# DmSM-1/C-OFDM

Hardware: AMD Instinct MI355X
Metric: IQ-samples/sec (tx IFFT+CP and rx FFT+equalise), 2048-subcarrier frames, 1/2/4/8 GPU (higher is better)
Workload: dtype f64

## Files before the change

c-ofdm_amd/csrc/ofdm_capi.cpp:

```cpp
#include <dlfcn.h>
#include <hip/hip_runtime.h>

#include <algorithm>
#include <climits>
#include <cctype>
#include <cmath>
#include <complex>
#include <cstdarg>
#include <cstdio>
#include <cstdlib>
#include <chrono>
#include <mutex>
#include <cstring>
#include <fstream>
#include <iterator>
#include <random>
#include <stdexcept>
#include <string>
#include <unordered_map>
#include <vector>

#include "../../include/ofdm_mi355x.h"

#if __has_include(<rccl/rccl.h>)
// ... 78 lines not shown
}

}

struct ofdm_ctx {
    ofdm_params p{};
    int device = 0;
    int logn = 0;
    int N = 0, D = 0, P = 0, cp = 0, S = 0, k = 0, L = 0, seg = 0, npr = 0, t2 = 0;
    ofdm_geometry geo{};
    std::vector<cd> t2_symbol, ofdm_preamble, mod_preamble, templ;
    std::vector<uint8_t> preamble_bytes;
    std::vector<double> t2_mask;
    double2* d_tw = nullptr;
    int* d_data_bin = nullptr;
    int* d_data_slot = nullptr;
    int* d_pilot_bin = nullptr;
    int* d_bin_map = nullptr;
    int* d_rx_pack = nullptr;
    int* d_pilot_swz = nullptr;
    int* d_tx_code = nullptr;
    double2* d_const = nullptr;
    double2* d_const_bpsk = nullptr;
    double2* d_header = nullptr;
    double2* d_preamble = nullptr;
    double2* d_templ = nullptr;
    double2* d_tspec = nullptr;
    float2* d_tspec32 = nullptr;
    double2* d_twm = nullptr;
    double tspec_max = 0.0;
    double2* d_modpre = nullptr;
    double* d_t2mask = nullptr;
    double2* d_t2tw = nullptr;
    int* d_first = nullptr;
    int t2_logn = -1;
    struct CfoPlan {
        int nsym = 0, logm = -1, g = 0;
        double2* tw_sub = nullptr;
        double2* tw_full = nullptr;
        int* borders = nullptr;
    };
    std::vector<CfoPlan> cfo_plans;
    double* d_cfo_scratch = nullptr;
    size_t cfo_scratch_n = 0;
    double2* d_scratch = nullptr;
    size_t scratch_bytes = 0;
// ... 278 lines not shown
                data_slot[d] = jj;
                bin_map[segst[jj] + t] = d;
            }
        }
    }
    std::vector<int> rx_pack(std::max(c->D, ofdm::RX_DPT * (c->N / 8)), 0),
        pilot_swz(std::max(c->P, c->N / 8), 0);
    for (int d = 0; d < c->D; ++d) rx_pack[d] = ofdm::lds_swz_host(data_bin[d]) | (data_slot[d] << 16);
    for (int j = 0; j < c->P; ++j) pilot_swz[j] = ofdm::lds_swz_host(pilot[j]);
    std::vector<int> tx_code(c->N);
    for (int b = 0; b < c->N; ++b)
        tx_code[b] = bin_map[b] >= 0 ? ofdm::tx_code_data(bin_map[b])
                                     : ofdm::tx_code_fixed(bin_map[b] == -2 ? ofdm::TX_LDS_PILOT : ofdm::TX_LDS_ZERO);
    if ((rc = upload(&c->d_rx_pack, rx_pack)) || (rc = upload(&c->d_pilot_swz, pilot_swz)) ||
        (rc = upload(&c->d_tx_code, tx_code)) ||
        (rc = upload(&c->d_tw, twiddles(c->N))) || (rc = upload(&c->d_data_bin, data_bin)) ||
        (rc = upload(&c->d_data_slot, data_slot)) || (rc = upload(&c->d_pilot_bin, pilot)) ||
        (rc = upload(&c->d_bin_map, bin_map)) || (rc = upload(&c->d_const, constellation(c->k))) ||
        (rc = upload(&c->d_const_bpsk, constellation(1)))) {
        ofdm_destroy(c);
        return rc;
    }

    c->t2_symbol.assign(c->t2, cd(0, 0));
    if (c->t2) {
        std::vector<cd> spec(c->t2, cd(0, 0));
        spec[params->t2_sin_f1] = cd(0.5, 0);
        spec[params->t2_sin_f2] = cd(0.5, 0);
        for (int n = 0; n < c->t2; ++n) {
            cd acc(0, 0);
            for (int kk = 0; kk < c->t2; ++kk) {
                if (spec[kk] == cd(0, 0)) continue;
                const double a = 2.0 * M_PI * (double)(((long)kk * n) % c->t2) / (double)c->t2;
                acc += spec[kk] * cd(std::cos(a), std::sin(a));
            }
            c->t2_symbol[n] = acc;
        }
    }
    c->t2_mask.assign(std::max(1, c->t2), 0.0);
    if (c->t2) {
        const int sm = (int)params->smooth, f1 = (int)params->t2_sin_f1, f2 = (int)params->t2_sin_f2;
        for (int i = std::max(0, f1 - sm); i <= std::min(c->t2 - 1, f1 + sm); ++i) c->t2_mask[i] += 1.0;
        for (int i = std::max(0, f2 - sm); i <= std::min(c->t2 - 1, f2 + sm); ++i) c->t2_mask[i] += 1.0;
    }

    {
// ... 193 lines not shown
    const int pilot_w = int(S * rel_pilot_w);
    std::vector<int> borders(P + 2);
    for (int i = 0, j = int((1.0 - rel_bw - rel_pilot_w) / 2.0 * S); i < P + 2; i++) {
        borders[i] = j;
        j += pilot_w;
    }
    borders[0] = std::max(0, borders[0]);
    for (int b : borders)
        if (b < 0 || b > S) return fail(OFDM_ERR_UNSUPPORTED, "pilot_freq_sinh windows leave the spectrum");
    int rc;
    if ((rc = upload(&pl.tw_sub, twiddles(1 << pl.logm))) || (rc = upload(&pl.borders, borders))) return rc;
    if (pl.g == 5 && (rc = upload(&pl.tw_full, twiddles((int)S)))) return rc;
    c->cfo_plans.push_back(pl);
    *out = &c->cfo_plans.back();
    return OFDM_OK;
}

int ofdm_get_geometry(const ofdm_ctx* c, ofdm_geometry* o)
{
    if (!c || !o) return fail(OFDM_ERR_INVALID, "null argument");
    *o = c->geo;
    return OFDM_OK;
}

int ofdm_get_t2_symbol(const ofdm_ctx* c, double* o)
{
    if (!c || !o) return fail(OFDM_ERR_INVALID, "null argument");
    std::memcpy(o, c->t2_symbol.data(), c->t2_symbol.size() * sizeof(cd));
    return OFDM_OK;
}

int ofdm_get_preamble(const ofdm_ctx* c, uint8_t* bytes, double* pre, double* modp, double* templ)
{
    if (!c) return fail(OFDM_ERR_INVALID, "null ctx");
    if (bytes) std::memcpy(bytes, c->preamble_bytes.data(), c->preamble_bytes.size());
    if (pre) std::memcpy(pre, c->ofdm_preamble.data(), c->ofdm_preamble.size() * sizeof(cd));
    if (modp) std::memcpy(modp, c->mod_preamble.data(), c->mod_preamble.size() * sizeof(cd));
    if (templ) std::memcpy(templ, c->templ.data(), c->templ.size() * sizeof(cd));
    return OFDM_OK;
}

int ofdm_device_alloc(ofdm_ctx* c, size_t bytes, void** d)
{
    if (!c || !d) return fail(OFDM_ERR_INVALID, "null argument");
    HIP_TRY(hipSetDevice(c->device));
    HIP_TRY(hipMalloc(d, std::max<size_t>(bytes, 1)));
// ... 205 lines not shown
    if (nframes > 0x7fffffffu) return fail(OFDM_ERR_INVALID, "too many frames in one call");
    ofdm::RxArgs a{};
    a.tab = c->tables(false);
    a.iq = iq16 ? nullptr : reinterpret_cast<const double2*>(iq);
    a.iq16 = reinterpret_cast<const short2*>(iq16);
    a.nframes = (long)nframes;
    a.frame_stride = (long)frame_stride;
    a.chan = reinterpret_cast<const double2*>(chan);
    a.chan_stride = (long)chan_stride;
    a.constell = reinterpret_cast<double2*>(constell_out);
    a.read_out = reinterpret_cast<double2*>(read_out);
    a.bytes = bytes_out;
    a.ref = ref_bytes;
    a.bit_errors = bit_errors;
    a.S = c->S;
    a.D = c->D;
    a.P = c->P;
    a.seg = c->seg;
    a.cp = c->cp;
    a.k = c->k;
    a.bytes_per_frame = c->geo.bytes_per_frame;
    a.pilot_ampl = (double)c->p.pilot_ampl / 1000;
    a.queue = rx_queue(c, (hipStream_t)stream);
    const bool fits = c->S <= ofdm::RX_SMAX && c->D <= ofdm::RX_DPT * (c->N / 8);
    if (!fits) {
        if (c->D > ofdm::RX_DPT * (c->N / 8))
            return fail(OFDM_ERR_UNSUPPORTED, "num_data_subc > fft_size/2 is not covered by the rx kernel");
        if (constell_out) {
            a.ystage = a.constell;
        } else {
            const size_t need = nframes * (size_t)c->S * c->D * sizeof(double2);
            if (need > c->scratch_bytes) {
                if (capturing((hipStream_t)stream)) return capture_refused("growing the staged rx scratch");
                HIP_TRY(hipSetDevice(c->device));
                if (c->d_scratch) HIP_TRY(hipFree(c->d_scratch));
                c->d_scratch = nullptr;
                c->scratch_bytes = 0;
                HIP_TRY(hipMalloc((void**)&c->d_scratch, need));
                c->scratch_bytes = need;
            }
            a.ystage = c->d_scratch;
        }
    }
    hipError_t e = soft ? ofdm::launch_rx_soft(c->logn, a, *soft, (hipStream_t)stream)
                        : ofdm::launch_rx(c->logn, a, (hipStream_t)stream, nullptr);
    if (e != hipSuccess) {
// ... 1429 lines not shown
```

c-ofdm_amd/csrc/ofdm_dev.hpp:

```cpp
#pragma once
#include <hip/hip_runtime.h>
#include <cstdint>
#include <mutex>
#include <set>
#include <utility>

#include "ofdm_fft.hpp"

namespace ofdm {

inline void lds_opt_in(const void* fn, int bytes)
{
    static std::mutex mu;
    static std::set<std::pair<const void*, int>> done;
    int dev = 0;
    if (hipGetDevice(&dev) != hipSuccess) dev = 0;
    std::lock_guard<std::mutex> g(mu);
    if (done.insert({fn, dev}).second)
        (void)hipFuncSetAttribute(fn, hipFuncAttributeMaxDynamicSharedMemorySize, bytes);
}

__device__ __forceinline__ int decide_select(double2 z, int k, double s1, int m)
{
    const double re = __builtin_fmin(__builtin_fmax(z.x, -1.0), 1.0);
    const double im = __builtin_fmin(__builtin_fmax(z.y, -1.0), 1.0);
    const int ire = (uint8_t)(int)add_rn(mul_rn(add_rn(re, 1.0), s1), 0.5);
    const int iim = (uint8_t)(int)add_rn(mul_rn(add_rn(im, 1.0), s1), 0.5);
    const int qam = (ire | (iim * m)) & 0xff;
    const int bpsk = (z.x + z.y) > 0.0;
    return k == 1 ? bpsk : qam;
}

enum { LLR_F32 = 0, LLR_I8 = 1 };

struct SoftScale {
    double c, h1;
    int h;
};

__device__ __forceinline__ SoftScale soft_scale(int k, double s)
{
    SoftScale q;
    q.h = k >> 1;
    q.h1 = (double)((1 << q.h) - 1) * 0.5;
    q.c = k == 1 ? -2.8284271247461903 * s : s / (q.h1 * q.h1);
    return q;
}

template <int H>
__device__ __forceinline__ void soft_axis(double x, double s1, const SoftScale& q, double (&L)[4])
{
#pragma unroll
    for (int b = 0; b < 4; ++b) L[b] = 0.0;
// ... 162 lines not shown
```

c-ofdm_amd/csrc/ofdm_internal.hpp:

```cpp
#pragma once
#include <hip/hip_runtime.h>
#include <cstdint>

namespace ofdm {

struct DevTables {
    const double2* tw;
    const int* data_bin;
    const int* data_slot;
    const int* pilot_bin;
    const int* bin_map;
    const int* rx_pack;
    const int* pilot_swz;
    const int* tx_code;
    const double2* constell;
};

struct TxArgs {
    DevTables tab;
    const uint8_t* bytes;
    const double2* points;
    double2* iq;
    int16_t* iq16;
    const double2* header;
// ... 17 lines not shown
struct RxArgs {
    DevTables tab;
    const double2* iq;
    const short2* iq16;
    long nframes;
    long frame_stride;
    const double2* chan;
    long chan_stride;
    bool chan_recip;
    double2* constell;
    double2* read_out;
    uint8_t* bytes;
    const uint8_t* ref;
    unsigned long long* bit_errors;
    double2* ystage;
    const long* starts;
    long start_off;
    const long* count;
    int* queue;
    const double2* corr;
    int S, D, P, seg, cp, k;
    long bytes_per_frame;
    double pilot_ampl;
};

struct SoftArgs {
    void* llr;
    const double* frame_scale;
    double scale;
    int fmt;
};

hipError_t launch_rx_soft(int logn, const RxArgs& a, const SoftArgs& sa, hipStream_t stream);
hipError_t launch_soft_demap(const double2* pts, long n, int k, double scale, int fmt, void* out, hipStream_t stream);
hipError_t launch_tx(int logn, const TxArgs& a, hipStream_t stream);
hipError_t launch_rx(int logn, const RxArgs& a, hipStream_t stream, bool* staged_needed);
hipError_t launch_copy(void* dst, const void* src, size_t n, hipStream_t stream);
hipError_t launch_demap(double2* pts, long n, int k, uint8_t* bytes, hipStream_t stream);
hipError_t launch_map(const uint8_t* bytes, long nbytes, int k, const double2* table, double2* out,
                      hipStream_t stream);
hipError_t launch_bit_convert(const uint8_t* in, long len, int in_bits, int out_bits, uint8_t* out, long out_len,
                              hipStream_t stream);
hipError_t launch_i16_to_f64(const int16_t* in, long n, double* out, hipStream_t stream);
hipError_t launch_f64_to_i16(const double* in, long n, double mult, int16_t* out, hipStream_t stream);

constexpr int RX_SMAX = 8;
inline int lds_swz_host(int e) { return e ^ ((e >> 3) & 7); }
constexpr int RX_DPT = 4;
constexpr int RX_WAVES_PER_CU = 8;
constexpr int TX_LDS_PILOT = 256, TX_LDS_ZERO = 257;
inline int tx_code_data(int d) { return d | (0xff << 13); }
inline int tx_code_fixed(int entry) { return entry << 21; }
constexpr long TX_MAX_GRID = 4096;


struct FecRate { int period, kept; unsigned mask; };
__host__ __device__ inline FecRate fec_rate(int rate)
{
    return rate == 0 ? FecRate{1, 1, 0x1u} : rate == 1 ? FecRate{4, 3, 0x7u} : FecRate{6, 4, 0x27u};
// ... 58 lines not shown
```

c-ofdm_amd/csrc/ofdm_kernels.hip:

```cpp
#include <hip/hip_runtime.h>
#include <algorithm>
#include <cstdint>
#include <cstdlib>

#include "ofdm_dev.hpp"
#include "ofdm_fft.hpp"
#include "ofdm_internal.hpp"
#include "ofdm_rx2.hpp"

#include <type_traits>

namespace ofdm {


__device__ __forceinline__ int symbol_bits(const uint8_t* __restrict__ b, long nbytes, long g, int k)
{
    const long bit = g * k;
    const long byte = bit >> 3;
    const int off = (int)(bit & 7);
    const int mask = (1 << k) - 1;
    if (off + k <= 8) return (b[byte] >> (8 - off - k)) & mask;
    const int w = ((int)b[byte] << 8) | (byte + 1 < nbytes ? (int)b[byte + 1] : 0);
    return (w >> (16 - off - k)) & mask;
}
// ... 798 lines not shown
            lds_opt_in((const void*)rx_wide_kernel<LOGN>, 160 * 1024);
            hipLaunchKernelGGL(rx_wide_kernel<LOGN>, dim3((unsigned)a.nframes), dim3(a.S * FS::T),
                               rx_wide_shm<LOGN>(a), st, a);
            return hipGetLastError();
        }
    }
    return fits ? rx_launch_n<LOGN, false, false, false>(a, st) : rx_launch_n<LOGN, true, false, false>(a, st);
}

hipError_t launch_rx(int logn, const RxArgs& a, hipStream_t st, bool* staged)
{
    switch (logn) {
        case 6: return rx_dispatch<6>(a, st, staged);
        case 7: return rx_dispatch<7>(a, st, staged);
        case 8: return rx_dispatch<8>(a, st, staged);
        case 9: return rx_dispatch<9>(a, st, staged);
        case 10: return rx_dispatch<10>(a, st, staged);
        case 11: return rx_dispatch<11>(a, st, staged);
        case 12: return rx_dispatch<12>(a, st, staged);
        default: return hipErrorInvalidValue;
    }
}

hipError_t launch_demap(double2* pts, long n, int k, uint8_t* bytes, hipStream_t st)
{
    const long nbytes = (n * k + 7) / 8;
    if (nbytes <= 0) return hipSuccess;
    const int bs = 256;
    hipLaunchKernelGGL(demap_kernel, dim3((unsigned)((nbytes + bs - 1) / bs)), dim3(bs), 0, st, pts, n, k, bytes,
                       nbytes);
    return hipGetLastError();
}

hipError_t launch_soft_demap(const double2* pts, long n, int k, double scale, int fmt, void* out, hipStream_t st)
{
    if (n <= 0) return hipSuccess;
    const long ntiles = (n + 1023) / 1024;
    const long cap = 8L * num_cus();
    const unsigned grid = (unsigned)(ntiles < cap ? ntiles : cap);
    if (fmt == LLR_F32)
        hipLaunchKernelGGL(soft_demap_kernel<LLR_F32>, dim3(grid), dim3(256), 0, st, pts, n, k, scale, out);
    else
        hipLaunchKernelGGL(soft_demap_kernel<LLR_I8>, dim3(grid), dim3(256), 0, st, pts, n, k, scale, out);
    return hipGetLastError();
}

// ... 113 lines not shown
```

c-ofdm_amd/csrc/ofdm_rx_body.inc:

```
    using FS = FftShape<LOGN>;
    constexpr int N = FS::N, T = FS::T;
    constexpr int SW = STAGED ? 1 : RX_SMAX;
    extern __shared__ double2 smem[];
    const int S0 = a.S, P0 = a.P;
    double2* bufA = smem;
    double2* bufB = bufA + N;
    double2* lds_tw = bufB + FS::PADN;
    double2* pil = lds_tw + TwLds<LOGN>::SIZE;
    double2* gain = pil + S0 * P0;
    double* red = reinterpret_cast<double*>(gain + S0 * P0);
    uint8_t* dec = reinterpret_cast<uint8_t*>(bufA);

    const int t0 = threadIdx.x;
    const int L = N + a.cp;
    const long fstep = gridDim.x;
    const long fbase = (SYNC && a.nframes > 0 && (!a.count || *a.count > 0) && a.starts[0] < 0) ? 1 : 0;
    const long nfr = (a.count ? min(*a.count, a.nframes) : a.nframes) - fbase;
    auto leave = [&]() {
        if (a.queue && threadIdx.x == 0) {
            __threadfence();
            if (atomicAdd(a.queue + 1, 1) == (int)gridDim.x - 1) {
                a.queue[0] = 0;
                a.queue[1] = 0;
            }
// ... 8 lines not shown
    constexpr bool kTwSplit = T >= TwLds<LOGN>::SIZE;
    TwPiece<LOGN> twp{};
    if constexpr (kTwSplit)
        twp = tw_fetch<LOGN>(a.tab.tw, t0);
    else
        load_twiddles<LOGN>(a.tab.tw, lds_tw, t0, T);
    int pk[RX_DPT];
#pragma unroll
    for (int i = 0; i < RX_DPT; ++i) pk[i] = a.tab.rx_pack[t0 + T * i];
    const int pbin = a.tab.pilot_swz[t0];
    long fl = blockIdx.x;
    auto frame_of = [&](long l) { return l + fbase; };
    SymbolRegs<LOGN, I16> pf;
    auto body0 = [&](long g) { return SYNC ? a.starts[g] + a.start_off : g * a.frame_stride + a.cp; };
    dma_symbol<LOGN, I16>(a, body0(frame_of(fl)), bufB, t0);
    if constexpr (kTwSplit) tw_store<LOGN>(twp, lds_tw);
    lds_barrier();

    unsigned long long errs = 0;

#pragma unroll 1
    for (long fnext; fl < nfr; fl = fnext) {
        const long f = frame_of(fl);
        int t;
        asm volatile("v_mov_b32 %0, %1" : "=v"(t) : "v"(t0));
#pragma unroll
        for (int i = 0; i < RX_DPT; ++i) asm volatile("" : "+v"(pk[i]));
        int S = a.S, D = a.D, P = a.P;
        asm volatile("" : "+s"(S), "+s"(D), "+s"(P));
        const long x0 = body0(f);
        const int m = 1 << (a.k / 2);
        const double s1 = a.k == 1 ? 0.0 : 1.0 / (2.0 / (m - 1));
        const bool whole_frame_dec = (long)S * D <= (long)FS::PADN * 16;
        const long bpf = a.bytes_per_frame;
        const bool by_word = (a.k == 1 || a.k == 2 || a.k == 4 || a.k == 8) && (bpf & 3) == 0 &&
                             ((uintptr_t)a.bytes & 3) == 0 && ((uintptr_t)a.ref & 3) == 0;
        SoftScale sq{};
        char* llr_f = nullptr;
        int llr_esz = 0;
        bool llr_vec = false;
        if constexpr (SOFT) {
            sq = soft_scale(a.k, sa.frame_scale ? sa.scale * sa.frame_scale[f] : sa.scale);
            llr_esz = sa.fmt == LLR_F32 ? 4 : 1;
            llr_f = static_cast<char*>(sa.llr) + f * S * D * a.k * llr_esz;
            llr_vec = ((uintptr_t)sa.llr & 15) == 0;
        }
// ... 36 lines not shown
            if (t < P) pil[s * P + t] = res[pbin];
            if constexpr (STAGED) {
#pragma unroll
                for (int i = 0; i < RX_DPT; ++i) {
                    const int d = t + T * i;
                    if (d < D) a.ystage[(f * S + s) * D + d] = res[pk[i] & 0xffff];
                }
            } else {
                switch (s) {
#define OFDM_RX_PUT(W)                                                                    \
    case W:                                                                               \
        if constexpr (W < SW) {                                                           \
            _Pragma("unroll") for (int i = 0; i < RX_DPT; ++i) y[W][i] = res[pk[i] & 0xffff]; \
        }                                                                                 \
        break;
                    OFDM_RX_PUT(0) OFDM_RX_PUT(1) OFDM_RX_PUT(2) OFDM_RX_PUT(3)
                    OFDM_RX_PUT(4) OFDM_RX_PUT(5) OFDM_RX_PUT(6) OFDM_RX_PUT(7)
#undef OFDM_RX_PUT
                    default: break;
                }
            }
        }
        lds_barrier();
        const double2* chan = a.chan ? a.chan + f * a.chan_stride : nullptr;
        const int dec_b = (S * D + 15) & ~15;
        double2* chl = reinterpret_cast<double2*>(reinterpret_cast<char*>(bufA) + dec_b);
        const bool chan_lds = chan && dec_b + D * 16 <= N * 16;
        if (chan_lds) dma_chan<LOGN>(chan, D, chl, t);
        const bool early = !a.queue;
        if (early) {
            fnext = fl + fstep;
            if (fnext < nfr) dma_symbol<LOGN, I16>(a, body0(frame_of(fnext)), bufB, t);
        }
        int qv = 0;
        if (a.queue && t == 0) qv = atomicAdd(a.queue, 1);

        double acc = 0.0;
        for (int i = t; i < S * P; i += T) acc += hypot(pil[i].x, pil[i].y);
        acc = block_sum_lds<T>(acc, red);
        const double phys = acc / ((double)(P * S) * a.pilot_ampl);

        for (int i = t; i < S * P; i += T) {
            const int j = i % P;
            const double2 c0 = make_double2(pil[j].x / phys, pil[j].y / phys);
            const double2 cs = make_double2(pil[i].x / phys, pil[i].y / phys);
            const double2 coef = cdiv_exact(cs, c0);
            const double2 g = cdiv_exact(make_double2(1.0, 0.0), coef);
            gain[i] = make_double2(g.x / phys, g.y / phys);
        }
        if (chan_lds) {
            if (early && fnext < nfr)
                asm volatile("s_waitcnt vmcnt(8)" ::: "memory");
            else
                asm volatile("s_waitcnt vmcnt(0)" ::: "memory");
        }
        if (a.queue && t == 0) *qslot = qv;
        lds_barrier();
        if (!early) {
            fnext = fstep + __builtin_amdgcn_readfirstlane(*qslot);
            if (fnext < nfr) dma_symbol<LOGN, I16>(a, body0(frame_of(fnext)), bufB, t);
        }

        auto emit_point = [&](int s, int i, double2 yv) {
            int d = t + T * i, gi = s * P + (pk[i] >> 16);
            asm volatile("" : "+v"(d), "+v"(gi));
            double2 o = cmul_exact(yv, gain[gi]);
            if (a.read_out) store_nt(a.read_out + (f * S + s) * D + d, o);
            const double2 cv = chan_lds ? chl[d] : load_untracked(chan + d);
            o = a.chan_recip ? cmul_exact(o, cv) : cdiv_exact(o, cv);
            if (a.constell) store_nt(a.constell + (f * S + s) * D + d, o);
            if constexpr (SOFT)
                soft_emit(o, a.k, s1, sq, sa.fmt, llr_f + (long)(s * D + d) * (a.k * llr_esz), llr_vec);
            dec[whole_frame_dec ? s * D + d : d] = (uint8_t)decide(o, a.k, s1, m);
// ... 2 lines not shown
            double2* cbase = a.constell + (f * S + s) * D;
#pragma unroll
            for (int i = 0; i < RX_DPT; ++i) {
                int d = t + T * i, gi = s * P + (pk[i] >> 16);
                asm volatile("" : "+v"(d), "+v"(gi));
                if (d < D) {
                    const double2 o = cmul_exact(yw[i], gain[gi]);
                    if constexpr (decltype(with_store)::value) store_nt(cbase + d, o);
                    if constexpr (SOFT)
                        soft_emit(o, a.k, s1, sq, sa.fmt, llr_f + (long)(s * D + d) * (a.k * llr_esz), llr_vec);
                    dec[whole_frame_dec ? s * D + d : d] = (uint8_t)decide_select(o, a.k, s1, m);
                }
            }
        };
        auto emit_group = [&](int s, const double2 (&yw)[RX_DPT]) {
            if (SYNC || chan) {
#pragma unroll
                for (int i = 0; i < RX_DPT; ++i)
                    if (t + T * i < D) emit_point(s, i, yw[i]);
            } else if (a.constell) {
                emit_plain(s, yw, std::true_type{});
            } else {
                emit_plain(s, yw, std::false_type{});
            }
        };

        auto pack = [&](long jb0, long jb1, long dbase) {
            for (long jb = jb0 + t; jb < jb1; jb += T) {
                int byte = 0;
                if (a.k == 1 || a.k == 2 || a.k == 4 || a.k == 8) {
                    const int per = 8 / a.k;
                    const long p0 = (jb - jb0) * per + dbase;
                    for (int r = 0; r < per; ++r) byte = (byte << a.k) | dec[p0 + r];
                } else {
                    for (int b = 0; b < 8; ++b) {
                        const long bit = (jb - jb0) * 8 + b;
                        const long g = bit / a.k + dbase;
                        const int within = (int)(bit % a.k);
                        byte = (byte << 1) | ((dec[g] >> (a.k - 1 - within)) & 1);
                    }
                }
                if (a.bytes) a.bytes[f * bpf + jb] = (uint8_t)byte;
                if (a.ref) errs += __popc((unsigned)(byte ^ a.ref[f * bpf + jb]));
            }
        };

        auto pack_words = [&]() {
            const int per_word = 32 / a.k;
            for (long w = t; w < bpf / 4; w += T) {
                const uint8_t* dw = dec + w * per_word;
                uint32_t word;
                switch (a.k) {
                    case 1: word = pack_word<1>(dw); break;
                    case 2: word = pack_word<2>(dw); break;
                    case 4: word = pack_word<4>(dw); break;
                    default: word = pack_word<8>(dw); break;
                }
                if (a.bytes) reinterpret_cast<uint32_t*>(a.bytes + f * bpf)[w] = word;
                if (a.ref) errs += __popc(word ^ reinterpret_cast<const uint32_t*>(a.ref + f * bpf)[w]);
            }
        };

        if constexpr (!STAGED) {
#pragma unroll 1
            for (int w = 0; w < S; ++w) {
                if constexpr (SOFT) {
                    double2 yw[RX_DPT] = {};
                    switch (w) {
#define OFDM_RX_TAKE(W)                                                        \
    case W:                                                                    \
        if constexpr (W < SW) {                                                \
            _Pragma("unroll") for (int i = 0; i < RX_DPT; ++i) yw[i] = y[W][i]; \
        }                                                                      \
        break;
                        OFDM_RX_TAKE(0) OFDM_RX_TAKE(1) OFDM_RX_TAKE(2) OFDM_RX_TAKE(3)
                        OFDM_RX_TAKE(4) OFDM_RX_TAKE(5) OFDM_RX_TAKE(6) OFDM_RX_TAKE(7)
#undef OFDM_RX_TAKE
                        default: break;
                    }
                    emit_group(w, yw);
                    continue;
                }
                switch (w) {
#define OFDM_RX_EMIT(W)                 \
    case W:                             \
        if constexpr (W < SW) {         \
            emit_group(w, y[W]);        \
        }                               \
        break;
                    OFDM_RX_EMIT(0) OFDM_RX_EMIT(1) OFDM_RX_EMIT(2) OFDM_RX_EMIT(3)
                    OFDM_RX_EMIT(4) OFDM_RX_EMIT(5) OFDM_RX_EMIT(6) OFDM_RX_EMIT(7)
#undef OFDM_RX_EMIT
                    default: break;
                }
            }
            lds_barrier();
            if (by_word)
                pack_words();
            else
                pack(0, bpf, 0);
        } else {
            const long bps = (long)D * a.k / 8;
            for (int s = 0; s < S; ++s) {
                double2 yst[RX_DPT];
#pragma unroll
                for (int i = 0; i < RX_DPT; ++i)
                    yst[i] = t + T * i < D ? a.ystage[(f * S + s) * D + t + T * i] : make_double2(0.0, 0.0);
                emit_group(s, yst);
                lds_barrier();
                if (!whole_frame_dec) {
                    pack(s * bps, (s + 1) * bps, 0);
                    lds_barrier();
                }
            }
            if (whole_frame_dec) pack(0, bpf, 0);
        }
        lds_barrier();
    }
    if (a.bit_errors) {
        errs = block_sum_u64<T>(errs, red);
        if (t0 == 0 && errs) atomicAdd(a.bit_errors, errs);
    }
    leave();
```

c-ofdm_amd/devtest/ofdm_devtest.hip:

```cpp
#include <hip/hip_runtime.h>

#include "../csrc/ofdm_syncdev.hpp"

namespace {

__global__ void atan2_kernel(const double* __restrict__ y, const double* __restrict__ x, double* __restrict__ out,
                             long n)
{
    const long i = (long)blockIdx.x * blockDim.x + threadIdx.x;
    if (i < n) out[i] = ofdm::atan2_fast(y[i], x[i]);
}

__global__ void cp_phase_kernel(const double2* __restrict__ acc, const double2* __restrict__ rot,
                                double* __restrict__ out, long n)
{
    const long i = (long)blockIdx.x * blockDim.x + threadIdx.x;
    if (i < n) out[i] = ofdm::cp_phase(acc[i], rot[i]);
}

template <int NT, bool WAVE>
__global__ void __launch_bounds__(WAVE ? 2 * NT : NT)
unwrap_kernel(double* __restrict__ ph, const int* __restrict__ len, long stride)
{
    __shared__ double lds[4 * NT + 1];
    __shared__ unsigned scr[(NT + 63) / 64];
    double* row = ph + (long)blockIdx.x * stride;
    const int n = min(len[blockIdx.x], 4 * NT + 1);
    for (int i = threadIdx.x; i < n; i += blockDim.x) lds[i] = row[i];
    __syncthreads();
    if (!WAVE || threadIdx.x < NT) ofdm::unwrap_scan<NT, WAVE>(lds, n, scr);
    __syncthreads();
    for (int i = threadIdx.x; i < n; i += blockDim.x) row[i] = lds[i];
}

template <int NT, bool WAVE>
int launch_unwrap(double* ph, const int* len, int nseq, long stride, hipStream_t s)
{
    hipLaunchKernelGGL((unwrap_kernel<NT, WAVE>), dim3(nseq), dim3(WAVE ? 2 * NT : NT), 0, s, ph, len, stride);
    return (int)hipGetLastError();
}

}

extern "C" {

int ofdm_devtest_atan2(const double* y, const double* x, double* out, long n, hipStream_t s)
{
    if (n <= 0) return 0;
    hipLaunchKernelGGL(atan2_kernel, dim3((unsigned)((n + 255) / 256)), dim3(256), 0, s, y, x, out, n);
    return (int)hipGetLastError();
}

int ofdm_devtest_cp_phase(const double* acc, const double* rot, double* out, long n, hipStream_t s)
{
    if (n <= 0) return 0;
    hipLaunchKernelGGL(cp_phase_kernel, dim3((unsigned)((n + 255) / 256)), dim3(256), 0, s,
                       reinterpret_cast<const double2*>(acc), reinterpret_cast<const double2*>(rot), out, n);
    return (int)hipGetLastError();
}

int ofdm_devtest_unwrap(int nt, int wave, double* ph, const int* len, int nseq, long stride, hipStream_t s)
{
    if (nseq <= 0) return 0;
    if (stride < 4L * nt + 1) return -1;
    if (wave) return nt == 64 ? launch_unwrap<64, true>(ph, len, nseq, stride, s) : -1;
    switch (nt) {
    case 8: return launch_unwrap<8, false>(ph, len, nseq, stride, s);
// ... 10 lines not shown
```

c-ofdm_amd/python/ofdm_mi355x.py:

```python
from __future__ import annotations

import ctypes as C
import os
import subprocess

HERE = os.path.dirname(os.path.abspath(__file__))
PKG = os.path.dirname(HERE)
LIB_PATH = os.environ.get("OFDM_MI355X_LIB") or os.path.join(PKG, "lib", "libofdm_mi355x.so")
HEADER = os.path.join(os.path.dirname(PKG), "include", "ofdm_mi355x.h")

PARAM_FIELDS = [
    "fft_size", "num_data_subc", "num_pilot_subc", "cp_size", "num_symb", "num_pr_symb",
    "pr_sin_len", "pr_seed", "pr_level", "t2sin_size", "t2_sin_f1", "t2_sin_f2",
    "t2_sin_level", "smooth", "mod_type", "pilot_ampl", "mult", "rx_buf_size", "iterations",
]

OFDM_OK = 0
ERRORS = {-1: "INVALID", -2: "UNSUPPORTED", -3: "HIP", -4: "IO", -5: "NOMEM", -6: "PARSE"}
LLR_F32, LLR_I8 = 0, 1
FEC_R12, FEC_R23, FEC_R34 = 0, 1, 2
IL_FORWARD, IL_INVERSE = 0, 1
SYNC_CFO, SYNC_FREQ_SHIFT, SYNC_CP, SYNC_PHASE, SYNC_CHAN, SYNC_ALL = 1, 2, 4, 8, 16, 31


# ... 30 lines not shown


class WalkState(C.Structure):
    _fields_ = [("pos", C.c_long), ("ring_end", C.c_long)]


class OfdmError(RuntimeError):
    def __init__(self, code: int, msg: str):
        super().__init__(f"ofdm error {code} ({ERRORS.get(code, '?')}): {msg}")
        self.code = code


_V, _I, _L, _SZ, _D = C.c_void_p, C.c_int, C.c_long, C.c_size_t, C.c_double
_PP = C.POINTER(Params)
SIGNATURES = {
    "ofdm_last_error": (C.c_char_p, []),
    "ofdm_abi_version": (_I, []),
    "ofdm_params_default": (_I, [_PP]),
    "ofdm_params_from_config": (_I, [C.c_char_p, _PP]),
    "ofdm_config_lookup": (_I, [C.c_char_p, C.c_char_p, C.POINTER(C.c_long)]),
    "ofdm_create": (_I, [_PP, _I, C.POINTER(_V)]),
    "ofdm_destroy": (_I, [_V]),
    "ofdm_get_geometry": (_I, [_V, C.POINTER(Geometry)]),
    "ofdm_get_t2_symbol": (_I, [_V, _V]),
    "ofdm_get_preamble": (_I, [_V, _V, _V, _V, _V]),
    "ofdm_device_alloc": (_I, [_V, _SZ, C.POINTER(_V)]),
    "ofdm_device_free": (_I, [_V, _V]),
    "ofdm_memcpy_h2d": (_I, [_V, _V, _V, _SZ, _V]),
    "ofdm_memcpy_d2h": (_I, [_V, _V, _V, _SZ, _V]),
    "ofdm_copy": (_I, [_V, _V, _V, _SZ, _V]),
    "ofdm_rx_demod_read": (_I, [_V, _V, _SZ, _SZ, _V, _SZ, _V, _V, _V, _V]),
    "ofdm_memset_device": (_I, [_V, _V, _I, _SZ, _V]),
    "ofdm_stream_synchronize": (_I, [_V, _V]),
    "ofdm_tx_modulate": (_I, [_V, _V, _SZ, _V, _SZ, _V, C.POINTER(Channel), _V]),
    "ofdm_tx_frames": (_I, [_V, _V, _SZ, _V, _V, _V]),
    "ofdm_rx_demod": (_I, [_V, _V, _SZ, _SZ, _V, _SZ, _V, _V, _V, _V, _V]),
    "ofdm_rx_demod_i16": (_I, [_V, _V, _SZ, _SZ, _V, _SZ, _V, _V, _V, _V, _V]),
    "ofdm_demap": (_I, [_V, _V, _SZ, _V, _V]),
    "ofdm_soft_demap": (_I, [_V, _V, _SZ, _D, _I, _V, _V]),
    "ofdm_rx_demod_soft": (_I, [_V, _V, _V, _SZ, _SZ, _V, _SZ, _D, _V, _I, _V, _V, _V, _V, _V, _V]),
    "ofdm_chan_estimate_ls": (_I, [_V, _V, _SZ, _SZ, _I, _V, _SZ, _V, _SZ, _V]),
    "ofdm_soft_demap_csi": (_I, [_V, _V, _SZ, _V, _SZ, _D, _V, _I, _V, _V]),
    "ofdm_fec_coded_bits": (_I, [_SZ, _I, C.POINTER(_SZ)]),
    "ofdm_fec_max_info_bits": (_I, [_SZ, _I, C.POINTER(_SZ)]),
    "ofdm_fec_workspace_size": (_I, [_SZ, _SZ, C.POINTER(_SZ)]),
    "ofdm_fec_encode": (_I, [_V, _V, _SZ, _SZ, _SZ, _I, _V, _SZ, _V]),
# ... 133 lines not shown
    def __init__(self, params, device: int = 0):
        if isinstance(params, dict):
            params = Params.make(**params)
        self.params = params
        self.device = device
        h = C.c_void_p()
        check(lib().ofdm_create(C.byref(params), device, C.byref(h)))
        self.h = h
        g = Geometry()
        check(lib().ofdm_get_geometry(h, C.byref(g)))
        self.geo = g

    def close(self):
        if getattr(self, "h", None):
            lib().ofdm_destroy(self.h)
            self.h = None

    def __del__(self):
        try:
            self.close()
        except Exception:
            pass

    def t2_symbol(self):
        import numpy as np
        out = np.zeros(self.params.t2sin_size, np.complex128)
        check(lib().ofdm_get_t2_symbol(self.h, out.ctypes.data))
        return out

    def preamble(self):
        import numpy as np
        p = self.params
        b = np.zeros(p.num_data_subc * p.num_pr_symb // 8, np.uint8)
        pre = np.zeros(self.geo.preamble_len, np.complex128)
        modp = np.zeros(p.num_data_subc * p.num_pr_symb, np.complex128)
        tpl = np.zeros(p.pr_sin_len, np.complex128)
        check(lib().ofdm_get_preamble(self.h, b.ctypes.data, pre.ctypes.data, modp.ctypes.data,
                                      tpl.ctypes.data))
        return b, pre, modp, tpl

    def tx(self, data, nframes: int, iq_out, frame_stride: int | None = None, iq16_out=None,
           noise_std: float = 0.0, seed: int = 0, sample_offset: int = 0, stream=None):
        stride = self.geo.message_len if frame_stride is None else frame_stride
        ch = Channel(noise_std, seed, sample_offset) if noise_std > 0 else None
        check(lib().ofdm_tx_modulate(self.h, _ptr(data), nframes, _ptr(iq_out), stride,
                                     _ptr(iq16_out), C.byref(ch) if ch else None, _stream(stream)))
# ... 237 lines not shown
```

include/ofdm_mi355x.h:

```cpp
#ifndef OFDM_MI355X_H
#define OFDM_MI355X_H

#include <stddef.h>
#include <stdint.h>

#ifdef __cplusplus
extern "C" {
#endif

#define OFDM_MI355X_ABI_VERSION 5

enum {
    OFDM_OK = 0,
    OFDM_ERR_INVALID = -1,
    OFDM_ERR_UNSUPPORTED = -2,
    OFDM_ERR_HIP = -3,
    OFDM_ERR_IO = -4,
    OFDM_ERR_NOMEM = -5,
    OFDM_ERR_PARSE = -6
};

typedef struct ofdm_params {
    long fft_size;
    long num_data_subc;
// ... 27 lines not shown
    long segment_size;
    long pilot_bin[256];
    long segment_bin[256];
} ofdm_geometry;

typedef struct ofdm_channel {
    double noise_std;
    unsigned long long seed;
    unsigned long long sample_offset;
} ofdm_channel;

typedef struct ofdm_ctx ofdm_ctx;

const char* ofdm_last_error(void);
int ofdm_abi_version(void);

int ofdm_params_default(ofdm_params* out);
int ofdm_params_from_config(const char* path, ofdm_params* out);
int ofdm_config_lookup(const char* path, const char* key, long* value);

int ofdm_create(const ofdm_params* params, int device, ofdm_ctx** out);
int ofdm_destroy(ofdm_ctx* ctx);
int ofdm_get_geometry(const ofdm_ctx* ctx, ofdm_geometry* out);
int ofdm_get_t2_symbol(const ofdm_ctx* ctx, double* out );
int ofdm_get_preamble(const ofdm_ctx* ctx,
                      uint8_t* bytes_out ,
                      double* ofdm_preamble_out ,
                      double* mod_preamble_out ,
                      double* template_out );

int ofdm_device_alloc(ofdm_ctx* ctx, size_t bytes, void** dptr);
int ofdm_device_free(ofdm_ctx* ctx, void* dptr);
int ofdm_memcpy_h2d(ofdm_ctx* ctx, void* dst, const void* src, size_t bytes, void* stream);
int ofdm_memcpy_d2h(ofdm_ctx* ctx, void* dst, const void* src, size_t bytes, void* stream);
int ofdm_memset_device(ofdm_ctx* ctx, void* dst, int value, size_t bytes, void* stream);
int ofdm_stream_synchronize(ofdm_ctx* ctx, void* stream);
int ofdm_host_alloc(ofdm_ctx* ctx, size_t bytes, void** hptr);
int ofdm_host_free(ofdm_ctx* ctx, void* hptr);
int ofdm_stream_create(ofdm_ctx* ctx, void** stream);
int ofdm_stream_destroy(ofdm_ctx* ctx, void* stream);
int ofdm_memcpy_d2d(ofdm_ctx* ctx, void* dst, const void* src, size_t bytes, void* stream);
int ofdm_copy(ofdm_ctx* ctx, void* dst, const void* src, size_t bytes, void* stream);
int ofdm_event_create(ofdm_ctx* ctx, void** event);
int ofdm_event_record(ofdm_ctx* ctx, void* event, void* stream);
int ofdm_event_synchronize(ofdm_ctx* ctx, void* event);
int ofdm_event_destroy(ofdm_ctx* ctx, void* event);
// ... 188 lines not shown
```

Before: 142.1 billion.

## Add fast QPSK rx emit path with threshold decisions and DPP word packing

Adds a fast receive emit path for QPSK without per-frame channel input. At create time a one-off device scan finds decision thresholds that match the existing decide_select bit for bit and validates them, then enables the path. In that path hard decisions become simple compares, and bits are packed into 32-bit words with cross-lane DPP moves and written directly, replacing the LDS staging, barrier and separate pack pass. Reference bytes are DMA'd into LDS for the bit-error count. This adds complexity and leaves the path off for other modulations or when validation fails.

```diff
diff --git a/c-ofdm_amd/csrc/ofdm_capi.cpp b/c-ofdm_amd/csrc/ofdm_capi.cpp
--- a/c-ofdm_amd/csrc/ofdm_capi.cpp
+++ b/c-ofdm_amd/csrc/ofdm_capi.cpp
@@ -124,6 +124,8 @@
     int* d_tx_code = nullptr;
     double2* d_const = nullptr;
     double2* d_const_bpsk = nullptr;
+    double dec_tau[3] = {};
+    bool dec_fast = false;
     double2* d_header = nullptr;
     double2* d_preamble = nullptr;
     double2* d_templ = nullptr;
@@ -448,6 +450,21 @@
         return rc;
     }
 
+    if (c->k == 2) {
+        double* d_tau = nullptr;
+        double h_tau[4] = {};
+        hipError_t e = hipMalloc((void**)&d_tau, sizeof(h_tau));
+        if (e == hipSuccess) e = ofdm::launch_decide_tau_scan(c->k, d_tau, nullptr);
+        if (e == hipSuccess) e = hipMemcpy(h_tau, d_tau, sizeof(h_tau), hipMemcpyDeviceToHost);
+        if (d_tau) (void)hipFree(d_tau);
+        if (e != hipSuccess) {
+            ofdm_destroy(c);
+            return hip_fail(e, "decision threshold scan");
+        }
+        for (int j = 0; j < 3; ++j) c->dec_tau[j] = h_tau[j];
+        c->dec_fast = h_tau[3] == 1.0;
+    }
+
     c->t2_symbol.assign(c->t2, cd(0, 0));
     if (c->t2) {
         std::vector<cd> spec(c->t2, cd(0, 0));
@@ -687,6 +704,8 @@
     *o = c->geo;
     return OFDM_OK;
 }
+
+int ofdm_rx_emit_fast(const ofdm_ctx* c) { return c ? (c->dec_fast ? 1 : 0) : -1; }
 
 int ofdm_get_t2_symbol(const ofdm_ctx* c, double* o)
 {
@@ -938,6 +957,8 @@
     a.bytes_per_frame = c->geo.bytes_per_frame;
     a.pilot_ampl = (double)c->p.pilot_ampl / 1000;
     a.queue = rx_queue(c, (hipStream_t)stream);
+    for (int j = 0; j < 3; ++j) a.dec_tau[j] = c->dec_tau[j];
+    a.dec_fast = c->dec_fast;
     const bool fits = c->S <= ofdm::RX_SMAX && c->D <= ofdm::RX_DPT * (c->N / 8);
     if (!fits) {
         if (c->D > ofdm::RX_DPT * (c->N / 8))
diff --git a/c-ofdm_amd/csrc/ofdm_dev.hpp b/c-ofdm_amd/csrc/ofdm_dev.hpp
--- a/c-ofdm_amd/csrc/ofdm_dev.hpp
+++ b/c-ofdm_amd/csrc/ofdm_dev.hpp
@@ -3,6 +3,7 @@
 #include <cstdint>
 #include <mutex>
 #include <set>
+#include <type_traits>
 #include <utility>
 
 #include "ofdm_fft.hpp"
@@ -29,6 +30,125 @@
     const int qam = (ire | (iim * m)) & 0xff;
     const int bpsk = (z.x + z.y) > 0.0;
     return k == 1 ? bpsk : qam;
+}
+
+constexpr int DEC_TAU_MAX = 3;
+
+template <int K>
+__device__ __forceinline__ unsigned axis_tau(double x, const double (&tau)[DEC_TAU_MAX])
+{
+    static_assert(K == 2 || K == 4, "thresholds cover QPSK and 16-QAM");
+    if constexpr (K == 2) {
+        return x >= tau[0] ? 1u : 0u;
+    } else {
+        const bool c0 = x >= tau[0], c1 = x >= tau[1], c2 = x >= tau[2];
+        return (c1 ? 2u : 0u) | ((c0 != c1) != c2 ? 1u : 0u);
+    }
+}
+
+template <int K>
+__device__ __forceinline__ unsigned decide_tau(double2 z, const double (&tau)[DEC_TAU_MAX])
+{
+    return axis_tau<K>(z.x, tau) | (axis_tau<K>(z.y, tau) << (K / 2));
+}
+
+__device__ __forceinline__ long long dbl_key(double x)
+{
+    const long long b = __double_as_longlong(x);
+    return b ^ ((b >> 63) & 0x7fffffffffffffffLL);
+}
+__device__ __forceinline__ double key_dbl(long long k)
+{
+    return __longlong_as_double(k ^ ((k >> 63) & 0x7fffffffffffffffLL));
+}
+
+__device__ __forceinline__ void decide_tau_scan(int k, double* __restrict__ out, double* lds)
+{
+    const int m = 1 << (k / 2);
+    const double s1 = 1.0 / (2.0 / (m - 1));
+    auto level = [&](double x) { return decide_select(make_double2(x, -1.0), k, s1, m) & (m - 1); };
+    const int t = threadIdx.x;
+    if (t == 0) {
+        bool ok = true;
+        for (int j = 1; j < DEC_TAU_MAX + 1; ++j) {
+            if (j >= m) {
+                lds[j - 1] = __longlong_as_double(0x7ff0000000000000LL);
+                continue;
+            }
+            const double edge = -1.0 + (double)(2 * j - 1) / (double)(m - 1);
+            long long lo = dbl_key(edge - 0.25), hi = dbl_key(edge + 0.25);
+            ok = ok && level(key_dbl(lo)) == j - 1 && level(key_dbl(hi)) == j;
+            while (hi - lo > 1) {
+                const long long mid = lo + (hi - lo) / 2;
+                if (level(key_dbl(mid)) >= j)
+                    hi = mid;
+                else
+                    lo = mid;
+            }
+            lds[j - 1] = key_dbl(hi);
+        }
+        lds[DEC_TAU_MAX] = ok ? 1.0 : 0.0;
+    }
+    __syncthreads();
+    double tau[DEC_TAU_MAX];
+    for (int j = 0; j < DEC_TAU_MAX; ++j) tau[j] = lds[j];
+    bool ok = lds[DEC_TAU_MAX] != 0.0;
+    auto same = [&](double x, double y) {
+        const double2 z = make_double2(x, y);
+        const unsigned want = (unsigned)decide_select(z, k, s1, m);
+        return want == (k == 2 ? decide_tau<2>(z, tau) : decide_tau<4>(z, tau));
+    };
+    for (int j = 0; j < m - 1; ++j) {
+        const long long c = dbl_key(tau[j]);
+        int prev = level(key_dbl(c - 1024 + t * 8 - 1));
+        for (int e = 0; e < 8; ++e) {
+            const double x = key_dbl(c - 1024 + t * 8 + e);
+            const int lv = level(x);
+            ok = ok && lv >= prev && same(x, -x) && same(-x, x);
+            prev = lv;
+        }
+    }
+    for (int i = t; i < 4096; i += 256) {
+        const double x = -1.5 + 3.0 * (double)i / 4095.0;
+        ok = ok && same(x, 0.3 - x) && level(x) <= level(x + 3.0 / 4095.0);
+    }
+    const double inf = __longlong_as_double(0x7ff0000000000000LL), qnan = __longlong_as_double(0x7ff8000000000000LL);
+    const double sp[16] = {0.0, -0.0, 1.0, -1.0, 1.0 + DBL_EPSILON, 1.0 - DBL_EPSILON / 2, -1.0 - DBL_EPSILON,
+                           -1.0 + DBL_EPSILON / 2, 2.0, -2.0, inf, -inf, qnan, -qnan, 0.5, -0.5};
+    ok = ok && same(sp[t & 15], sp[(t >> 4) & 15]);
+    const int all = __syncthreads_and(ok ? 1 : 0);
+    if (t == 0) {
+        for (int j = 0; j < DEC_TAU_MAX; ++j) out[j] = tau[j];
+        out[DEC_TAU_MAX] = all ? 1.0 : 0.0;
+    }
+}
+
+template <int K>
+__device__ __forceinline__ bool emit_collects(int lane)
+{
+    return ((lane / (8 / K)) & 3) == 3;
+}
+
+template <int K>
+__device__ __forceinline__ void emit_words(unsigned bits, int lane, unsigned (&w)[K / 2])
+{
+    constexpr int LPB = 8 / K;
+    auto dpp = [](unsigned x, auto ctrl) {
+        return (unsigned)__builtin_amdgcn_update_dpp(0, (int)x, decltype(ctrl)::value, 0xf, 0xf, true);
+    };
+    const int r = lane & (LPB - 1);
+    unsigned v = bits << (K * (LPB - 1 - r));
+    v |= dpp(v, std::integral_constant<int, 0xB1>{});
+    if constexpr (LPB == 4) v |= dpp(v, std::integral_constant<int, 0x4E>{});
+    const int q = (lane / LPB) & 3;
+#pragma unroll
+    for (int h = 0; h < K / 2; ++h) {
+        const int g = r + LPB * h;
+        const unsigned b = ((v >> (8 * g)) & 0xffu) << (8 * q);
+        w[h] = b | dpp(b, std::integral_constant<int, 0x110 + LPB>{})
+                 | dpp(b, std::integral_constant<int, 0x110 + 2 * LPB>{})
+                 | dpp(b, std::integral_constant<int, 0x110 + 3 * LPB>{});
+    }
 }
 
 enum { LLR_F32 = 0, LLR_I8 = 1 };
diff --git a/c-ofdm_amd/csrc/ofdm_internal.hpp b/c-ofdm_amd/csrc/ofdm_internal.hpp
--- a/c-ofdm_amd/csrc/ofdm_internal.hpp
+++ b/c-ofdm_amd/csrc/ofdm_internal.hpp
@@ -63,6 +63,8 @@
     int S, D, P, seg, cp, k;
     long bytes_per_frame;
     double pilot_ampl;
+    double dec_tau[3];
+    int dec_fast;
 };
 
 struct SoftArgs {
@@ -76,6 +78,7 @@
 hipError_t launch_soft_demap(const double2* pts, long n, int k, double scale, int fmt, void* out, hipStream_t stream);
 hipError_t launch_tx(int logn, const TxArgs& a, hipStream_t stream);
 hipError_t launch_rx(int logn, const RxArgs& a, hipStream_t stream, bool* staged_needed);
+hipError_t launch_decide_tau_scan(int k, double* out, hipStream_t stream);
 hipError_t launch_copy(void* dst, const void* src, size_t n, hipStream_t stream);
 hipError_t launch_demap(double2* pts, long n, int k, uint8_t* bytes, hipStream_t stream);
 hipError_t launch_map(const uint8_t* bytes, long nbytes, int k, const double2* table, double2* out,
diff --git a/c-ofdm_amd/csrc/ofdm_kernels.hip b/c-ofdm_amd/csrc/ofdm_kernels.hip
--- a/c-ofdm_amd/csrc/ofdm_kernels.hip
+++ b/c-ofdm_amd/csrc/ofdm_kernels.hip
@@ -844,6 +844,19 @@
     }
 }
 
+__global__ void __launch_bounds__(256) decide_tau_scan_kernel(int k, double* out)
+{
+    __shared__ double lds[DEC_TAU_MAX + 1];
+    decide_tau_scan(k, out, lds);
+}
+
+hipError_t launch_decide_tau_scan(int k, double* out, hipStream_t st)
+{
+    if (k != 2 && k != 4) return hipErrorInvalidValue;
+    hipLaunchKernelGGL(decide_tau_scan_kernel, dim3(1), dim3(256), 0, st, k, out);
+    return hipGetLastError();
+}
+
 hipError_t launch_demap(double2* pts, long n, int k, uint8_t* bytes, hipStream_t st)
 {
     const long nbytes = (n * k + 7) / 8;
diff --git a/c-ofdm_amd/csrc/ofdm_rx_body.inc b/c-ofdm_amd/csrc/ofdm_rx_body.inc
--- a/c-ofdm_amd/csrc/ofdm_rx_body.inc
+++ b/c-ofdm_amd/csrc/ofdm_rx_body.inc
@@ -54,6 +54,7 @@
 #pragma unroll 1
     for (long fnext; fl < nfr; fl = fnext) {
         const long f = frame_of(fl);
+        OFDM_PHASE(rx_symbols);
         int t;
         asm volatile("v_mov_b32 %0, %1" : "=v"(t) : "v"(t0));
 #pragma unroll
@@ -136,11 +137,21 @@
             }
         }
         lds_barrier();
+        OFDM_PHASE(rx_phys_gains);
         const double2* chan = a.chan ? a.chan + f * a.chan_stride : nullptr;
         const int dec_b = (S * D + 15) & ~15;
         double2* chl = reinterpret_cast<double2*>(reinterpret_cast<char*>(bufA) + dec_b);
         const bool chan_lds = chan && dec_b + D * 16 <= N * 16;
         if (chan_lds) dma_chan<LOGN>(chan, D, chl, t);
+        bool fast = false;
+        if constexpr (!SOFT && !STAGED && !SYNC && T >= 64)
+            fast = a.dec_fast && !chan && a.k == 2 && (D & 63) == 0 && by_word &&
+                   ((uintptr_t)a.ref & 15) == 0;
+        uint8_t* refl = reinterpret_cast<uint8_t*>(bufA);
+        const bool ref_lds = fast && a.ref;
+        if (ref_lds)
+            dma_chan<LOGN>(reinterpret_cast<const double2*>(a.ref + f * bpf), (int)(bpf >> 4),
+                           reinterpret_cast<double2*>(refl), t);
         const bool early = !a.queue;
         if (early) {
             fnext = fl + fstep;
@@ -162,7 +173,7 @@
             const double2 g = cdiv_exact(make_double2(1.0, 0.0), coef);
             gain[i] = make_double2(g.x / phys, g.y / phys);
         }
-        if (chan_lds) {
+        if (chan_lds || ref_lds) {
             if (early && fnext < nfr)
                 asm volatile("s_waitcnt vmcnt(8)" ::: "memory");
             else
@@ -211,6 +222,46 @@
                 emit_plain(s, yw, std::true_type{});
             } else {
                 emit_plain(s, yw, std::false_type{});
+            }
+        };
+
+        auto emit_fast = [&](int s, const double2 (&yw)[RX_DPT], auto kc) {
+            constexpr int K = decltype(kc)::value, LPB = 8 / K;
+            const double tau[DEC_TAU_MAX] = {a.dec_tau[0], a.dec_tau[1], a.dec_tau[2]};
+            int tt;
+            asm volatile("v_mov_b32 %0, %1" : "=v"(tt) : "v"(t));
+            const int lane = tt & 63;
+            const int w0 = __builtin_amdgcn_readfirstlane(tt & ~63);
+            const int na = w0 < D ? min((D - w0 + T - 1) / T, RX_DPT) : 0;
+            double2* cbase = a.constell + (f * S + s) * D;
+            double2 gv[RX_DPT];
+#pragma unroll
+            for (int i = 0; i < RX_DPT; ++i) {
+                int gi = s * P + (pk[i] >> 16);
+                asm volatile("" : "+v"(gi));
+                gv[i] = gain[gi];
+            }
+            unsigned bits = 0;
+#pragma unroll
+            for (int i = 0; i < RX_DPT; ++i) {
+                const double2 o = cmul_exact(yw[i], gv[i]);
+                int d = tt + T * i;
+                asm volatile("" : "+v"(d));
+                if (a.constell && i < na) store_nt(cbase + d, o);
+                bits |= decide_tau<K>(o, tau) << (8 * i);
+            }
+            unsigned w[K / 2];
+            emit_words<K>(bits, lane, w);
+            if (emit_collects<K>(lane)) {
+#pragma unroll
+                for (int h = 0; h < K / 2; ++h) {
+                    const int g = (lane & (LPB - 1)) + LPB * h;
+                    if (g < na) {
+                        const int off = (((s * D + w0 + T * g) * K) >> 3) + 4 * (lane / (4 * LPB));
+                        if (a.bytes) *reinterpret_cast<uint32_t*>(a.bytes + f * bpf + off) = w[h];
+                        if (a.ref) errs += __popc(w[h] ^ *reinterpret_cast<const uint32_t*>(refl + off));
+                    }
+                }
             }
         };
 
@@ -250,7 +301,27 @@
             }
         };
 
-        if constexpr (!STAGED) {
+        if (fast) {
+            if constexpr (!SOFT && !STAGED && !SYNC && T >= 64) {
+                OFDM_PHASE(rx_emit_fast);
+#pragma unroll 1
+                for (int w = 0; w < S; ++w) {
+                    switch (w) {
+#define OFDM_RX_FAST(W)                                           \
+    case W:                                                       \
+        if constexpr (W < SW) {                                   \
+            emit_fast(w, y[W], std::integral_constant<int, 2>{}); \
+        }                                                         \
+        break;
+                        OFDM_RX_FAST(0) OFDM_RX_FAST(1) OFDM_RX_FAST(2) OFDM_RX_FAST(3)
+                        OFDM_RX_FAST(4) OFDM_RX_FAST(5) OFDM_RX_FAST(6) OFDM_RX_FAST(7)
+#undef OFDM_RX_FAST
+                        default: break;
+                    }
+                }
+            }
+        } else if constexpr (!STAGED) {
+            OFDM_PHASE(rx_emit);
 #pragma unroll 1
             for (int w = 0; w < S; ++w) {
                 if constexpr (SOFT) {
@@ -284,11 +355,13 @@
                 }
             }
             lds_barrier();
+            OFDM_PHASE(rx_pack);
             if (by_word)
                 pack_words();
             else
                 pack(0, bpf, 0);
         } else {
+            OFDM_PHASE(rx_emit);
             const long bps = (long)D * a.k / 8;
             for (int s = 0; s < S; ++s) {
                 double2 yst[RX_DPT];
@@ -304,8 +377,10 @@
             }
             if (whole_frame_dec) pack(0, bpf, 0);
         }
+        OFDM_PHASE(rx_frame_end);
         lds_barrier();
     }
+    OFDM_PHASE(rx_end);
     if (a.bit_errors) {
         errs = block_sum_u64<T>(errs, red);
         if (t0 == 0 && errs) atomicAdd(a.bit_errors, errs);
diff --git a/c-ofdm_amd/devtest/ofdm_devtest.hip b/c-ofdm_amd/devtest/ofdm_devtest.hip
--- a/c-ofdm_amd/devtest/ofdm_devtest.hip
+++ b/c-ofdm_amd/devtest/ofdm_devtest.hip
@@ -1,5 +1,6 @@
 #include <hip/hip_runtime.h>
 
+#include "../csrc/ofdm_dev.hpp"
 #include "../csrc/ofdm_syncdev.hpp"
 
 namespace {
@@ -40,9 +41,70 @@
     return (int)hipGetLastError();
 }
 
+__global__ void __launch_bounds__(256) tau_scan_kernel(int k, double* out)
+{
+    __shared__ double lds[ofdm::DEC_TAU_MAX + 1];
+    ofdm::decide_tau_scan(k, out, lds);
+}
+
+template <int K>
+__global__ void decide_kernel(const double2* __restrict__ z, const double* __restrict__ tau,
+                              uint8_t* __restrict__ sel, uint8_t* __restrict__ thr, long n)
+{
+    const long i = (long)blockIdx.x * blockDim.x + threadIdx.x;
+    if (i >= n) return;
+    const int m = 1 << (K / 2);
+    const double s1 = 1.0 / (2.0 / (m - 1));
+    const double t[ofdm::DEC_TAU_MAX] = {tau[0], tau[1], tau[2]};
+    sel[i] = (uint8_t)ofdm::decide_select(z[i], K, s1, m);
+    thr[i] = (uint8_t)ofdm::decide_tau<K>(z[i], t);
+}
+
+template <int K>
+__global__ void __launch_bounds__(64) emit_words_kernel(const unsigned* __restrict__ bits,
+                                                        unsigned* __restrict__ words)
+{
+    const long i = (long)blockIdx.x * 64 + threadIdx.x;
+    unsigned w[K / 2];
+    ofdm::emit_words<K>(bits[i], (int)threadIdx.x, w);
+    for (int h = 0; h < K / 2; ++h) words[2 * i + h] = w[h];
+}
+
 }
 
 extern "C" {
+
+int ofdm_devtest_tau_scan(int k, double* out, hipStream_t s)
+{
+    if (k != 2 && k != 4) return -1;
+    hipLaunchKernelGGL(tau_scan_kernel, dim3(1), dim3(256), 0, s, k, out);
+    return (int)hipGetLastError();
+}
+
+int ofdm_devtest_decide(int k, const double* z, const double* tau, uint8_t* sel, uint8_t* thr, long n,
+                        hipStream_t s)
+{
+    if (k != 2 && k != 4) return -1;
+    if (n <= 0) return 0;
+    const dim3 grid((unsigned)((n + 255) / 256));
+    const double2* zz = reinterpret_cast<const double2*>(z);
+    if (k == 2)
+        hipLaunchKernelGGL(decide_kernel<2>, grid, dim3(256), 0, s, zz, tau, sel, thr, n);
+    else
+        hipLaunchKernelGGL(decide_kernel<4>, grid, dim3(256), 0, s, zz, tau, sel, thr, n);
+    return (int)hipGetLastError();
+}
+
+int ofdm_devtest_emit_words(int k, const unsigned* bits, unsigned* words, int nwaves, hipStream_t s)
+{
+    if (k != 2 && k != 4) return -1;
+    if (nwaves <= 0) return 0;
+    if (k == 2)
+        hipLaunchKernelGGL(emit_words_kernel<2>, dim3(nwaves), dim3(64), 0, s, bits, words);
+    else
+        hipLaunchKernelGGL(emit_words_kernel<4>, dim3(nwaves), dim3(64), 0, s, bits, words);
+    return (int)hipGetLastError();
+}
 
 int ofdm_devtest_atan2(const double* y, const double* x, double* out, long n, hipStream_t s)
 {
diff --git a/c-ofdm_amd/python/ofdm_mi355x.py b/c-ofdm_amd/python/ofdm_mi355x.py
--- a/c-ofdm_amd/python/ofdm_mi355x.py
+++ b/c-ofdm_amd/python/ofdm_mi355x.py
@@ -76,6 +76,7 @@
     "ofdm_create": (_I, [_PP, _I, C.POINTER(_V)]),
     "ofdm_destroy": (_I, [_V]),
     "ofdm_get_geometry": (_I, [_V, C.POINTER(Geometry)]),
+    "ofdm_rx_emit_fast": (_I, [_V]),
     "ofdm_get_t2_symbol": (_I, [_V, _V]),
     "ofdm_get_preamble": (_I, [_V, _V, _V, _V, _V]),
     "ofdm_device_alloc": (_I, [_V, _SZ, C.POINTER(_V)]),
@@ -255,6 +256,9 @@
         except Exception:
             pass
 
+    def rx_emit_fast(self) -> bool:
+        return lib().ofdm_rx_emit_fast(self.h) == 1
+
     def t2_symbol(self):
         import numpy as np
         out = np.zeros(self.params.t2sin_size, np.complex128)
diff --git a/include/ofdm_mi355x.h b/include/ofdm_mi355x.h
--- a/include/ofdm_mi355x.h
+++ b/include/ofdm_mi355x.h
@@ -73,6 +73,7 @@
 int ofdm_create(const ofdm_params* params, int device, ofdm_ctx** out);
 int ofdm_destroy(ofdm_ctx* ctx);
 int ofdm_get_geometry(const ofdm_ctx* ctx, ofdm_geometry* out);
+int ofdm_rx_emit_fast(const ofdm_ctx* ctx);
 int ofdm_get_t2_symbol(const ofdm_ctx* ctx, double* out );
 int ofdm_get_preamble(const ofdm_ctx* ctx,
                       uint8_t* bytes_out ,
```

New measurement: 144.3 billion (median of 6 runs). 1.02x the previous value.
